# kaiidams/voice100

Measured on AMD Instinct MI355X. Metric: audio frames/sec (fwd+bwd) asr_en_base, B=32x1024-frame mel, higher is better.
Workload: dtype bf16

## Files before the change

voice100_amd/csrc/ctc.hip:

```cpp
#include "common.h"
#include <math.h>
#include <type_traits>

#define CTC_CHUNK 64
#define CTC_MAXV 128
#define NEG_INF (-INFINITY)

__device__ __forceinline__ float lse2(float a, float b) {
    const float m = fmaxf(a, b);
    if (m == NEG_INF) return NEG_INF;
    return m + __logf(__expf(a - m) + __expf(b - m));
}
__device__ __forceinline__ float lse3(float a, float b, float c) {
    const float m = fmaxf(fmaxf(a, b), c);
    if (m == NEG_INF) return NEG_INF;
    return m + __logf(__expf(a - m) + __expf(b - m) + __expf(c - m));
}

__global__ void ctc_lse_kernel(const float* __restrict__ logits, float* __restrict__ lse, long rows, int V, int* __restrict__ stall, int B) {
    const long r = (long)blockIdx.x * blockDim.x + threadIdx.x;
    if (r < B) stall[r] = 0;
    if (r >= rows) return;
    const float* p = logits + r * V;
    float m = NEG_INF;
    for (int c = 0; c < V; ++c) m = fmaxf(m, p[c]);
    float s = 0.f;
    for (int c = 0; c < V; ++c) s += expf(p[c] - m);
    lse[r] = m + logf(s);
}

template <int NS>
__global__ __launch_bounds__(256) void ctc_lattice_kernel(const float* __restrict__ logits, const float* __restrict__ lse,
                                                          const long long* __restrict__ targets, const int* __restrict__ in_len,
                                                          const int* __restrict__ tgt_len, float* __restrict__ alpha,
                                                          float* __restrict__ beta, float* __restrict__ nll, int T, int V, int Lmax,
                                                          int Smax, int blank) {
    extern __shared__ float sm[];
    float* lp = sm;
    float* row = sm + CTC_CHUNK * V;
    const int b = blockIdx.x, dir = blockIdx.y, tid = threadIdx.x;
    int Tb = in_len[b];
    if (Tb > T) Tb = T;
    int L = tgt_len[b];
    if (L > Lmax) L = Lmax;
    const int S = 2 * L + 1;
    float* lat = (dir == 0 ? alpha : beta) + (size_t)b * T * Smax;
    const long long* tg = targets + (size_t)b * Lmax;
    const int rs = Smax + 4;
    for (int i = tid; i < 2 * rs; i += 256) row[i] = NEG_INF;
    __syncthreads();
    if (Tb <= 0) { if (dir == 0 && tid == 0) nll[b] = INFINITY; return; }

    int cls[NS]; bool skip[NS];
#pragma unroll
    for (int k = 0; k < NS; ++k) {
        const int s = tid + 256 * k;
        cls[k] = blank; skip[k] = false;
        if (s < S && (s & 1)) {
            cls[k] = (int)tg[s >> 1];
            if (dir == 0) skip[k] = s >= 2 && tg[s >> 1] != tg[(s >> 1) - 1];
            else skip[k] = s + 2 < S && tg[s >> 1] != tg[(s >> 1) + 1];
        }
        if (cls[k] < 0 || cls[k] >= V) cls[k] = blank;
    }

    const int nchunks = (Tb + CTC_CHUNK - 1) / CTC_CHUNK;
    for (int ci = 0; ci < nchunks; ++ci) {
        const int c0 = dir == 0 ? ci * CTC_CHUNK : (nchunks - 1 - ci) * CTC_CHUNK;
        const int cn = min(CTC_CHUNK, Tb - c0);
        __syncthreads();
        for (int i = tid; i < cn * V; i += 256) {
            const int tt = i / V, c = i - tt * V;
            lp[i] = logits[((size_t)b * T + c0 + tt) * V + c] - lse[(size_t)b * T + c0 + tt];
        }
        __syncthreads();
        for (int j = 0; j < cn; ++j) {
            const int tl = dir == 0 ? j : cn - 1 - j;
            const int t = c0 + tl;
            const bool first = dir == 0 ? (t == 0) : (t == Tb - 1);
            const int cur = t & 1, prv = cur ^ 1;
#pragma unroll
            for (int k = 0; k < NS; ++k) {
                const int s = tid + 256 * k;
                if (s < S) {
                    const float e = lp[tl * V + cls[k]];
                    float v;
                    if (first) {
                        const bool start = dir == 0 ? (s <= 1) : (s >= S - 2);
                        v = start ? e : NEG_INF;
                    } else if (dir == 0) {
                        const float* pr = row + prv * rs + 2 + s;
                        v = e + lse3(pr[0], pr[-1], skip[k] ? pr[-2] : NEG_INF);
                    } else {
                        const float* pr = row + prv * rs + 2 + s;
                        v = e + lse3(pr[0], pr[1], skip[k] ? pr[2] : NEG_INF);
                    }
                    row[cur * rs + 2 + s] = v;
                    lat[(size_t)t * Smax + s] = v;
                }
            }
            __syncthreads();
        }
    }
    if (dir == 0 && tid == 0) {
        const float* last = row + ((Tb - 1) & 1) * rs + 2;
        const float ll = S >= 2 ? lse2(last[S - 1], last[S - 2]) : last[S - 1];
        nll[b] = -ll;
    }
}

__device__ __forceinline__ float ctc_lse3_log2(float a, float b, float c) {
    const float mm = fmaxf(fmaxf(fmaxf(a, b), c), -1e30f);
    const float sum = __builtin_amdgcn_exp2f(a - mm) + __builtin_amdgcn_exp2f(b - mm) + __builtin_amdgcn_exp2f(c - mm);
    return mm + __builtin_amdgcn_logf(sum);
}
#define CTC_RING 32
#define CTC_SPIN_MAX (1 << 20)
#define CTC_PF 8
__device__ __forceinline__ float ctc_wave_shr1(float fill, float v) {
    return __builtin_bit_cast(float, __builtin_amdgcn_update_dpp(__builtin_bit_cast(int, fill), __builtin_bit_cast(int, v), 0x138, 0xf, 0xf, false));
}

__global__ __launch_bounds__(1024) void ctc_lattice_skew_kernel(const float* __restrict__ logits, const float* __restrict__ lse,
                                                                const long long* __restrict__ targets, const int* __restrict__ in_len,
                                                                const int* __restrict__ tgt_len, float* __restrict__ alpha,
                                                                float* __restrict__ beta, float* __restrict__ nll, int T, int V, int Lmax,
                                                                int Smax, int blank, int* __restrict__ stall) {
    __shared__ float bnd[16][CTC_RING][2];
    __shared__ int progress[16];
    __shared__ float fin[2];
    const int b = blockIdx.x, dir = blockIdx.y, tid = threadIdx.x;
    const int w = __builtin_amdgcn_readfirstlane(tid >> 6), lane = tid & 63, NW = blockDim.x >> 6;
    int Tb = in_len[b];
    if (Tb > T) Tb = T;
    int L = tgt_len[b];
    if (L > Lmax) L = Lmax;
    const int S = 2 * L + 1;
    float* lat = (dir == 0 ? alpha : beta) + (size_t)b * T * Smax;
    const long long* tg = targets + (size_t)b * Lmax;
    if (lane == 0) progress[w] = -1;
    if (tid < 2) fin[tid] = NEG_INF;
    __syncthreads();
    if (Tb <= 0) { if (dir == 0 && tid == 0) nll[b] = INFINITY; return; }

    const int u = tid;
    const int sidx = dir == 0 ? u : S - 1 - u;
    const bool active = u < S;
    int cls = blank;
    bool skip = false;
    if (active && (sidx & 1)) {
        cls = (int)tg[sidx >> 1];
        if (dir == 0) skip = sidx >= 2 && tg[sidx >> 1] != tg[(sidx >> 1) - 1];
        else skip = sidx + 2 < S && tg[sidx >> 1] != tg[(sidx >> 1) + 1];
    }
    if (cls < 0 || cls >= V) cls = blank;

    const float* lg = logits + (size_t)b * T * V + cls;
    const float* ls = lse + (size_t)b * T;
    auto emission = [&](int q) -> float {
        const int qq = q < Tb ? q : Tb - 1;
        const int t = dir == 0 ? qq : Tb - 1 - qq;
        return (lg[(size_t)t * V] - ls[t]) * 1.44269504088896340736f;
    };
    float cur[CTC_PF], nxt[CTC_PF];
#pragma unroll
    for (int j = 0; j < CTC_PF; ++j) cur[j] = emission(j);

    auto prog_load = [&](int i) { return __hip_atomic_load(&progress[i], __ATOMIC_RELAXED, __HIP_MEMORY_SCOPE_WORKGROUP); };
    float a_prev = NEG_INF;
    int pnext = -2;
    float n63 = NEG_INF, n62 = NEG_INF;
    float* lrow = lat + (size_t)(dir == 0 ? 0 : Tb - 1) * Smax + sidx;
    const long lstep = dir == 0 ? (long)Smax : -(long)Smax;
    auto frame = [&](auto up_t, auto down_t, auto first_t, int q, float e) {
        constexpr bool UP = decltype(up_t)::value, DOWN = decltype(down_t)::value, FIRST = decltype(first_t)::value;
        float v63 = NEG_INF, v62 = NEG_INF;
        if constexpr (UP) {
            if constexpr (!FIRST) {
                asm volatile("" : "+v"(pnext));
                if (__builtin_amdgcn_readfirstlane(pnext) >= q - 1) {
                    v63 = n63; v62 = n62;
                } else {
                    const int need = min(q + 1, Tb - 1);
                    int guard = 0;
                    for (; prog_load(w - 1) < need && guard < CTC_SPIN_MAX; ++guard) __builtin_amdgcn_s_sleep(1);
                    if (guard >= CTC_SPIN_MAX && lane == 0) stall[b] = 1;
                    asm volatile("" ::: "memory");
                    v63 = bnd[w - 1][(q - 1) & (CTC_RING - 1)][0];
                    v62 = bnd[w - 1][(q - 1) & (CTC_RING - 1)][1];
                }
            }
            pnext = prog_load(w - 1);
            asm volatile("" ::: "memory");
            n63 = bnd[w - 1][q & (CTC_RING - 1)][0];
            n62 = bnd[w - 1][q & (CTC_RING - 1)][1];
        }
        float v;
        if constexpr (FIRST) {
            v = (u <= 1) ? e : NEG_INF;
        } else {
            const float sm1 = ctc_wave_shr1(v63, a_prev);
            const float sm2 = ctc_wave_shr1(v62, sm1);
            v = e + ctc_lse3_log2(a_prev, sm1, skip ? sm2 : NEG_INF);
        }
        if (!active) v = NEG_INF;
        if constexpr (DOWN) {
            if ((q & (CTC_RING / 2 - 1)) == 0 && q >= CTC_RING / 2) {
                int guard = 0;
                for (; prog_load(w + 1) < q - CTC_RING / 2 && guard < CTC_SPIN_MAX; ++guard) __builtin_amdgcn_s_sleep(1);
                if (guard >= CTC_SPIN_MAX && lane == 0) stall[b] = 1;
            }
            asm volatile("" ::: "memory");
            if (lane >= 62) bnd[w][q & (CTC_RING - 1)][63 - lane] = v;
        }
        asm volatile("" ::: "memory");
        if (lane == 0) __hip_atomic_store(&progress[w], q, __ATOMIC_RELAXED, __HIP_MEMORY_SCOPE_WORKGROUP);
        a_prev = v;
        if (active) *lrow = v * 0.69314718055994530942f;
        lrow += lstep;
    };
    auto run = [&](auto up_t, auto down_t) {
        for (int q0 = 0; q0 < Tb; q0 += CTC_PF) {
#pragma unroll
            for (int j = 0; j < CTC_PF; ++j) nxt[j] = emission(q0 + CTC_PF + j);
            if (q0 == 0) {
                frame(up_t, down_t, std::true_type{}, 0, cur[0]);
#pragma unroll
                for (int j = 1; j < CTC_PF; ++j)
                    if (j < Tb) frame(up_t, down_t, std::false_type{}, j, cur[j]);
            } else if (q0 + CTC_PF <= Tb) {
#pragma unroll
                for (int j = 0; j < CTC_PF; ++j) frame(up_t, down_t, std::false_type{}, q0 + j, cur[j]);
            } else {
#pragma unroll
                for (int j = 0; j < CTC_PF; ++j)
                    if (q0 + j < Tb) frame(up_t, down_t, std::false_type{}, q0 + j, cur[j]);
            }
#pragma unroll
            for (int j = 0; j < CTC_PF; ++j) cur[j] = nxt[j];
        }
    };
    const bool has_up = w > 0, has_down = w < NW - 1;
    if (has_up && has_down) run(std::true_type{}, std::true_type{});
    else if (has_up) run(std::true_type{}, std::false_type{});
    else if (has_down) run(std::false_type{}, std::true_type{});
    else run(std::false_type{}, std::false_type{});
    if (dir == 0) {
        if (u == S - 1) fin[0] = a_prev;
        if (S >= 2 && u == S - 2) fin[1] = a_prev;
        __syncthreads();
        if (tid == 0) nll[b] = -(S >= 2 ? lse2(fin[0] * 0.69314718055994530942f, fin[1] * 0.69314718055994530942f) : fin[0] * 0.69314718055994530942f);
    }
}

template <int NW, bool BVT>
__global__ __launch_bounds__(64 * NW) void ctc_grad_kernel(const float* __restrict__ logits, const float* __restrict__ lse,
                                                           const long long* __restrict__ targets, const int* __restrict__ in_len,
                                                           const int* __restrict__ tgt_len, const float* __restrict__ alpha,
                                                           const float* __restrict__ beta, float* nll,
                                                           float* __restrict__ grad, int B, int T, int V, int Lmax, int Smax, int blank,
                                                           int mean_scale, const int* __restrict__ stall, float* __restrict__ loss) {
    __shared__ float bins[2 * NW][CTC_MAXV];
    __shared__ float stage[BVT ? NW : 1][BVT ? CTC_MAXV : 1];
    const int wave = threadIdx.x >> 6, lane = threadIdx.x & 63;
    const long w = (long)blockIdx.x * NW + wave;
    if (loss && blockIdx.x == 0 && wave == 0) {
        float s = 0.f;
        for (int bb = lane; bb < B; bb += 64) {
            const float v = stall[bb] ? __builtin_nanf("") : nll[bb];
            if (!(v == INFINITY || v == -INFINITY)) s += v / (float)max(tgt_len[bb], 1);
        }
        s = wave_sum(s);
        if (lane == 0) loss[0] = s / (float)B;
    }
    const auto frame = [&]() {
    const int b = (int)(w / T), t = (int)(w % T);
    float* g = BVT ? &stage[wave][0] : grad + ((size_t)b * T + t) * V;
    if (stall[b]) {
        for (int c = lane; c < V; c += 64) g[c] = __builtin_nanf("");
        if (t == 0 && lane == 0) nll[b] = __builtin_nanf("");
        return;
    }
    const float n = nll[b];
    int Tb = in_len[b];
    if (Tb > T) Tb = T;
    if (t >= Tb || !(n < INFINITY)) {
        for (int c = lane; c < V; c += 64) g[c] = 0.f;
        return;
    }
    int L = tgt_len[b];
    if (L > Lmax) L = Lmax;
    const int S = 2 * L + 1;
    const float* al = alpha + ((size_t)b * T + t) * Smax;
    const float* be = beta + ((size_t)b * T + t) * Smax;
    const long long* tg = targets + (size_t)b * Lmax;
    unsigned* dmin = reinterpret_cast<unsigned*>(&bins[NW + wave][0]);
    for (int c = lane; c < V; c += 64) { bins[wave][c] = 0.f; dmin[c] = 0x7f800000u; }
    float m = NEG_INF;
    for (int s = lane; s < S; s += 64) m = fmaxf(m, al[s] + be[s]);
#pragma unroll
    for (int off = 32; off > 0; off >>= 1) m = fmaxf(m, __shfl_xor(m, off, 64));
    __builtin_amdgcn_wave_barrier();
    asm volatile("" ::: "memory");
    if (m > NEG_INF) {
        for (int s = lane; s < S; s += 64) {
            int c = (s & 1) ? (int)tg[s >> 1] : blank;
            if (c < 0 || c >= V) c = blank;
            const float d = m - (al[s] + be[s]);
            if (d >= 0.f) atomicMin(&dmin[c], __builtin_bit_cast(unsigned, d));
        }
        __builtin_amdgcn_wave_barrier();
        asm volatile("" ::: "memory");
        for (int s = lane; s < S; s += 64) {
            int c = (s & 1) ? (int)tg[s >> 1] : blank;
            if (c < 0 || c >= V) c = blank;
            const float dm = __builtin_bit_cast(float, dmin[c]);
            const float x = al[s] + be[s];
            if (dm < INFINITY || x != x) atomicAdd(&bins[wave][c], expf((x - m) + dm));
        }
    }
    __builtin_amdgcn_wave_barrier();
    asm volatile("" ::: "memory");
    const float z = lse[(size_t)b * T + t];
    const float* lg = logits + ((size_t)b * T + t) * V;
    const float gs = mean_scale ? 1.f / ((float)max(tgt_len[b], 1) * (float)B) : 1.f;
    for (int c = lane; c < V; c += 64) {
        const float lpc = lg[c] - z;
        const float acc = bins[wave][c];
        const float dm = __builtin_bit_cast(float, dmin[c]);
        const float occ = (acc > 0.f) ? expf(((m - dm) + n - lpc) + logf(acc)) : (acc != acc ? acc : 0.f);
        g[c] = (expf(lpc) - occ) * gs;
    }
    };
    if (w < (long)B * T) frame();
    if constexpr (BVT) {
        __syncthreads();
        const long w0 = (long)blockIdx.x * NW;
        for (int i = threadIdx.x; i < V * NW; i += 64 * NW) {
            const int c = i / NW, j = i % NW;
            const long wj = w0 + j;
            if (wj < (long)B * T) grad[((size_t)(wj / T) * V + c) * T + (wj % T)] = stage[j][c];
        }
    }
}

extern "C" int v100_ctc_workspace_floats(int B, int T, int Lmax) {
    const long n = 2L * B * T * (2 * Lmax + 1) + (long)B * T + B;
    return n > 0x7fffffffL ? -1 : (int)n;
}

static int ctc_run(const float* logits, const long long* targets, const int* in_len, const int* tgt_len, float* workspace, float* nll,
                   float* loss, float* grad, int grad_bvt, int B, int T, int V, int Lmax, int blank, void* stream);

extern "C" int v100_ctc_loss(const float* logits, const long long* targets, const int* in_len, const int* tgt_len, float* workspace,
                             float* nll, float* grad, int B, int T, int V, int Lmax, int blank, void* stream) {
    return ctc_run(logits, targets, in_len, tgt_len, workspace, nll, nullptr, grad, 0, B, T, V, Lmax, blank, stream);
}

extern "C" int v100_ctc_loss_mean(const float* logits, const long long* targets, const int* in_len, const int* tgt_len, float* workspace,
                                  float* nll, float* loss, float* grad, int B, int T, int V, int Lmax, int blank, void* stream) {
    if (!loss) return V100_ERR_NULL;
    return ctc_run(logits, targets, in_len, tgt_len, workspace, nll, loss, grad, 0, B, T, V, Lmax, blank, stream);
}

extern "C" int v100_ctc_loss_mean_t(const float* logits, const long long* targets, const int* in_len, const int* tgt_len,
                                    float* workspace, float* nll, float* loss, float* grad, int grad_bvt, int B, int T, int V, int Lmax,
                                    int blank, void* stream) {
    if (!loss) return V100_ERR_NULL;
    return ctc_run(logits, targets, in_len, tgt_len, workspace, nll, loss, grad, grad_bvt ? 1 : 0, B, T, V, Lmax, blank, stream);
}

static int ctc_run(const float* logits, const long long* targets, const int* in_len, const int* tgt_len, float* workspace, float* nll,
                   float* loss, float* grad, int grad_bvt, int B, int T, int V, int Lmax, int blank, void* stream) {
    if (!logits || !targets || !in_len || !tgt_len || !workspace || !nll || !grad) return V100_ERR_NULL;
    if (B <= 0 || T <= 0 || V <= 0 || V > CTC_MAXV || Lmax < 0 || 2 * Lmax + 1 > 4096 || blank < 0 || blank >= V) return V100_ERR_SHAPE;
    hipStream_t st = (hipStream_t)stream;
    const int Smax = 2 * Lmax + 1;
    float* alpha = workspace;
    float* beta = alpha + (size_t)B * T * Smax;
    float* lse = beta + (size_t)B * T * Smax;
    const long rows = (long)B * T;
    int* stall = (int*)(lse + (size_t)B * T);
    V100_GGL(ctc_lse_kernel, dim3((unsigned)((rows + 255) / 256)), dim3(256), 0, st, logits, lse, rows, V, stall, B);
    const size_t shmem = (size_t)(CTC_CHUNK * V + 2 * (Smax + 4)) * sizeof(float);
#define CTC_LATTICE(NS_)                                                                                                          \
    if (shmem > 65536)                                                                                                            \
        (void)hipFuncSetAttribute((const void*)ctc_lattice_kernel<NS_>, hipFuncAttributeMaxDynamicSharedMemorySize, (int)shmem);       \
    V100_GGL(ctc_lattice_kernel<NS_>, dim3(B, 2), dim3(256), shmem, st, logits, lse, targets, in_len, tgt_len, alpha, beta, \
                       nll, T, V, Lmax, Smax, blank)
    if (Smax <= 1024) {
        const int nw = (Smax + 63) / 64;
        V100_GGL(ctc_lattice_skew_kernel, dim3(B, 2), dim3(64 * nw), 0, st, logits, lse, targets, in_len, tgt_len, alpha, beta,
                           nll, T, V, Lmax, Smax, blank, stall);
    } else if (Smax <= 2048) { CTC_LATTICE(8); }
    else { CTC_LATTICE(16); }
#undef CTC_LATTICE
    if (grad_bvt) V100_GGL((ctc_grad_kernel<16, true>), dim3((unsigned)((rows + 15) / 16)), dim3(1024), 0, st, logits, lse, targets, in_len, tgt_len,
                           alpha, beta, nll, grad, B, T, V, Lmax, Smax, blank, loss ? 1 : 0, stall, loss);
    else V100_GGL((ctc_grad_kernel<4, false>), dim3((unsigned)((rows + 3) / 4)), dim3(256), 0, st, logits, lse, targets, in_len, tgt_len,
                  alpha, beta, nll, grad, B, T, V, Lmax, Smax, blank, loss ? 1 : 0, stall, loss);
    return v100_launch_status();
}
```

Before: 10.38 million.

## Add halo-overlap CTC lattice kernel syncing waves every K frames

Adds a CTC alpha/beta lattice kernel in which each 64-lane wave recomputes a halo of 2K overlapping states. Neighbouring waves exchange boundary values through a shared-memory ring only once every K frames, instead of handing off the skew every frame. It is meant to cut per-frame inter-wave synchronisation latency on the sequential time recurrence. In exchange it does redundant halo computation, uses more waves per block, and adds spin-wait and stall-detection complexity. It is enabled by default when the wave count fits in 16, and an environment variable can turn it off.

```diff
diff --git a/voice100_amd/csrc/ctc.hip b/voice100_amd/csrc/ctc.hip
--- a/voice100_amd/csrc/ctc.hip
+++ b/voice100_amd/csrc/ctc.hip
@@ -1,5 +1,6 @@
 #include "common.h"
 #include <math.h>
+#include <stdlib.h>
 #include <type_traits>
 
 #define CTC_CHUNK 64
@@ -253,6 +254,150 @@
     }
 }
 
+#define CTC_HALO_K 4
+#define CTC_HALO_RING 8
+template <int K>
+__global__ __launch_bounds__(1024) void ctc_lattice_halo_kernel(const float* __restrict__ logits, const float* __restrict__ lse,
+                                                                const long long* __restrict__ targets, const int* __restrict__ in_len,
+                                                                const int* __restrict__ tgt_len, float* __restrict__ alpha,
+                                                                float* __restrict__ beta, float* __restrict__ nll, int T, int V, int Lmax,
+                                                                int Smax, int blank, int* __restrict__ stall) {
+    constexpr int H = 2 * K, P = 64 - H, RING = CTC_HALO_RING;
+    static_assert(K >= 2 && (K & (K - 1)) == 0 && P >= H, "a wave's halo must come from ONE neighbour: 64 - 2 K >= 2 K");
+    static_assert(K <= CTC_PF ? CTC_PF % K == 0 : K % CTC_PF == 0, "block boundaries fall on fixed frames of a prefetch group");
+    __shared__ float edge[16][RING][H];
+    __shared__ int progress[16];
+    __shared__ float fin[2];
+    const int b = blockIdx.x, dir = blockIdx.y, tid = threadIdx.x;
+    const int w = __builtin_amdgcn_readfirstlane(tid >> 6), lane = tid & 63, NW = blockDim.x >> 6;
+    int Tb = in_len[b];
+    if (Tb > T) Tb = T;
+    int L = tgt_len[b];
+    if (L > Lmax) L = Lmax;
+    const int S = 2 * L + 1;
+    float* lat = (dir == 0 ? alpha : beta) + (size_t)b * T * Smax;
+    const long long* tg = targets + (size_t)b * Lmax;
+    if (lane == 0) progress[w] = -1;
+    if (tid < 2) fin[tid] = NEG_INF;
+    __syncthreads();
+    if (Tb <= 0) { if (dir == 0 && tid == 0) nll[b] = INFINITY; return; }
+
+    const int u = w * P - H + lane;
+    const bool active = u >= 0 && u < S;
+    const bool owned = active && lane >= H;
+    const int sidx = active ? (dir == 0 ? u : S - 1 - u) : 0;
+    int cls = blank;
+    bool skip = false;
+    if (active && (sidx & 1)) {
+        cls = (int)tg[sidx >> 1];
+        if (dir == 0) skip = sidx >= 2 && tg[sidx >> 1] != tg[(sidx >> 1) - 1];
+        else skip = sidx + 2 < S && tg[sidx >> 1] != tg[(sidx >> 1) + 1];
+    }
+    if (cls < 0 || cls >= V) cls = blank;
+
+    const float* lg = logits + (size_t)b * T * V + cls;
+    const float* ls = lse + (size_t)b * T;
+    auto emission = [&](int q) -> float {
+        const int qq = q < Tb ? q : Tb - 1;
+        const int t = dir == 0 ? qq : Tb - 1 - qq;
+        return (lg[(size_t)t * V] - ls[t]) * 1.44269504088896340736f;
+    };
+    float cur[CTC_PF], nxt[CTC_PF];
+#pragma unroll
+    for (int j = 0; j < CTC_PF; ++j) cur[j] = emission(j);
+
+    auto prog_load = [&](int i) { return __hip_atomic_load(&progress[i], __ATOMIC_RELAXED, __HIP_MEMORY_SCOPE_WORKGROUP); };
+    float a_prev = NEG_INF;
+    float* lrow = lat + (size_t)(dir == 0 ? 0 : Tb - 1) * Smax + sidx;
+    const long lstep = dir == 0 ? (long)Smax : -(long)Smax;
+    auto frame = [&](auto up_t, auto down_t, auto first_t, bool blast, int q, float e) {
+        constexpr bool UP = decltype(up_t)::value, DOWN = decltype(down_t)::value, FIRST = decltype(first_t)::value;
+        const int n = q / K;
+        int pn = 0;
+        float hv = NEG_INF;
+        if constexpr (UP) {
+            if (blast) {
+                pn = prog_load(w - 1);
+                asm volatile("" ::: "memory");
+                hv = edge[w - 1][n & (RING - 1)][lane & (H - 1)];
+            }
+        }
+        float v;
+        if constexpr (FIRST) {
+            v = (u == 0 || u == 1) ? e : NEG_INF;
+        } else {
+            const float sm1 = ctc_wave_shr1(NEG_INF, a_prev);
+            const float sm2 = ctc_wave_shr1(NEG_INF, sm1);
+            v = e + ctc_lse3_log2(a_prev, sm1, skip ? sm2 : NEG_INF);
+        }
+        if (!active) v = NEG_INF;
+        if (blast) {
+            if constexpr (DOWN) {
+                if ((n & (RING / 2 - 1)) == 0 && n >= RING / 2) {
+                    int guard = 0;
+                    for (; prog_load(w + 1) < n - RING / 2 && guard < CTC_SPIN_MAX; ++guard) __builtin_amdgcn_s_sleep(1);
+                    if (guard >= CTC_SPIN_MAX && lane == 0) stall[b] = 1;
+                }
+                asm volatile("" ::: "memory");
+                if (lane >= 64 - H) edge[w][n & (RING - 1)][lane - (64 - H)] = v;
+            }
+            asm volatile("" ::: "memory");
+            if (lane == 0) __hip_atomic_store(&progress[w], n, __ATOMIC_RELAXED, __HIP_MEMORY_SCOPE_WORKGROUP);
+        }
+        a_prev = v;
+        if (owned) *lrow = v * 0.69314718055994530942f;
+        lrow += lstep;
+        if constexpr (UP) {
+            if (blast) {
+                asm volatile("" : "+v"(pn));
+                if (__builtin_amdgcn_readfirstlane(pn) < n) {
+                    int guard = 0;
+                    for (; prog_load(w - 1) < n && guard < CTC_SPIN_MAX; ++guard) __builtin_amdgcn_s_sleep(1);
+                    if (guard >= CTC_SPIN_MAX && lane == 0) stall[b] = 1;
+                    asm volatile("" ::: "memory");
+                    hv = edge[w - 1][n & (RING - 1)][lane & (H - 1)];
+                }
+                if (lane < H) a_prev = hv;
+            }
+        }
+    };
+    auto run = [&](auto up_t, auto down_t) {
+        for (int q0 = 0; q0 < Tb; q0 += CTC_PF) {
+#pragma unroll
+            for (int j = 0; j < CTC_PF; ++j) nxt[j] = emission(q0 + CTC_PF + j);
+            const bool g_last = (q0 & (K - 1)) == K - CTC_PF;
+#define bl(j) (K <= CTC_PF ? (j) % K == K - 1 : ((j) == CTC_PF - 1 && g_last))
+            if (q0 == 0) {
+                frame(up_t, down_t, std::true_type{}, false, 0, cur[0]);
+#pragma unroll
+                for (int j = 1; j < CTC_PF; ++j)
+                    if (j < Tb) frame(up_t, down_t, std::false_type{}, bl(j), j, cur[j]);
+            } else if (q0 + CTC_PF <= Tb) {
+#pragma unroll
+                for (int j = 0; j < CTC_PF; ++j) frame(up_t, down_t, std::false_type{}, bl(j), q0 + j, cur[j]);
+            } else {
+#pragma unroll
+                for (int j = 0; j < CTC_PF; ++j)
+                    if (q0 + j < Tb) frame(up_t, down_t, std::false_type{}, bl(j), q0 + j, cur[j]);
+            }
+#undef bl
+#pragma unroll
+            for (int j = 0; j < CTC_PF; ++j) cur[j] = nxt[j];
+        }
+    };
+    const bool has_up = w > 0, has_down = w < NW - 1;
+    if (has_up && has_down) run(std::true_type{}, std::true_type{});
+    else if (has_up) run(std::true_type{}, std::false_type{});
+    else if (has_down) run(std::false_type{}, std::true_type{});
+    else run(std::false_type{}, std::false_type{});
+    if (dir == 0) {
+        if (owned && u == S - 1) fin[0] = a_prev;
+        if (owned && S >= 2 && u == S - 2) fin[1] = a_prev;
+        __syncthreads();
+        if (tid == 0) nll[b] = -(S >= 2 ? lse2(fin[0] * 0.69314718055994530942f, fin[1] * 0.69314718055994530942f) : fin[0] * 0.69314718055994530942f);
+    }
+}
+
 template <int NW, bool BVT>
 __global__ __launch_bounds__(64 * NW) void ctc_grad_kernel(const float* __restrict__ logits, const float* __restrict__ lse,
                                                            const long long* __restrict__ targets, const int* __restrict__ in_len,
@@ -388,7 +533,13 @@
         (void)hipFuncSetAttribute((const void*)ctc_lattice_kernel<NS_>, hipFuncAttributeMaxDynamicSharedMemorySize, (int)shmem);       \
     V100_GGL(ctc_lattice_kernel<NS_>, dim3(B, 2), dim3(256), shmem, st, logits, lse, targets, in_len, tgt_len, alpha, beta, \
                        nll, T, V, Lmax, Smax, blank)
-    if (Smax <= 1024) {
+    const char* halo = getenv("V100_CTC_HALO");
+    constexpr int HALO_P = 64 - 2 * CTC_HALO_K;
+    const int nwh = (Smax + HALO_P - 1) / HALO_P;
+    if (nwh <= 16 && !(halo && halo[0] == '0')) {
+        V100_GGL(ctc_lattice_halo_kernel<CTC_HALO_K>, dim3(B, 2), dim3(64 * nwh), 0, st, logits, lse, targets, in_len, tgt_len, alpha,
+                 beta, nll, T, V, Lmax, Smax, blank, stall);
+    } else if (Smax <= 1024) {
         const int nw = (Smax + 63) / 64;
         V100_GGL(ctc_lattice_skew_kernel, dim3(B, 2), dim3(64 * nw), 0, st, logits, lse, targets, in_len, tgt_len, alpha, beta,
                            nll, T, V, Lmax, Smax, blank, stall);
```

New measurement: 10.49 million, median of 5. About the same (+1.0%).
